# raynbowy23/RegT-GCN

Hardware: AMD Instinct MI355X
Metric: training steps/sec (graph-snapshots/sec) (higher is better)
Workload: dtype fp32; 1 GPU; cfg3: ONE synthetic regional graph, 100000 nodes / 1000000 edges / 8 regions, F=32, T=12, O=1, hidden=256; RegionalTemporalGCN forward+MSE+backward per snapshot, RMSprop step once per K steps (run.py semantics); gemm_arithmetic=fp32 MFMA (v_mfma_f32_32x32x2_f32), global_nodes=100000, global_edges=1000000, global_regions=8, parallelism=single GPU

## Files before the change

regt-gcn_amd/csrc/api.hip:

```cpp
#include <limits.h>
#include <stdarg.h>

#include <functional>
#include <initializer_list>
#include <map>
#include <mutex>
#include <string>
#include <unordered_map>
#include <vector>

#include "../../include/regtgcn.h"
#include <algorithm>
#include "kernels.h"

namespace regt {

static thread_local char g_err[512] = "";
void set_error(const char* fmt, ...) {
    va_list ap;
    va_start(ap, fmt);
    vsnprintf(g_err, sizeof(g_err), fmt, ap);
    va_end(ap);
}

// ... 976 lines not shown
    TRY(rq.flush());
    PROF("compose_bwd", st);
    {
        SgBatch b{};
        for (int k = 0; k < 3; ++k) {
            const float* dG = k < 2 ? L.dGzr + (long)k * C * F : L.dGh;
            const float* dc = k < 2 ? L.dczr + (long)k * C : L.dch;
            add_task(b, gr.gate_w[k], 2L * C, 1, 0, C, C, 1, nullptr, 0,
                     {term(dG, F, 1, 0, p.conv_lin_w[k], 1, F, 0, F), term(dc, 1, 0, 0, p.conv_bias[k], 0, 1, 0, 1)});
            add_task(b, gr.conv_lin_w[k], 1, F, 0, F, C, 1, nullptr, 0, {term(dG, 1, F, 0, p.gate_w[k], 2L * C, 1, 0, C)});
            add_task(b, gr.conv_bias[k], 1, 0, 0, C, 1, 1, nullptr, 0, {term(p.gate_w[k], 1, 2L * C, 0, dc, 1, 0, 0, C)});
        }
        for (int k = 0; k < 3; ++k)
            add_task(b, gr.gate_b[k], 1, 0, 0, C, 1, 1, k < 2 ? L.dczr + (long)k * C : L.dch, 1, {});
        if (tcol) {
            const float* dP0[2] = {L.dP01, L.dP01 + (long)C * 2 * F};
            const float* dP1[2] = {L.dP01 + F, L.dP01 + (long)C * 2 * F + F};
            const float* dc[2] = {L.dczr, L.dczr + C};
            for (int k = 0; k < 2; ++k)
                add_task(b, gr.gate_w[k] + C, 2L * C, 1, 0, C, C, 1, nullptr, 0,
                         {term(dP0[k], 2L * F, 1, 0, p.cheb_w0, 1, F, 0, F), term(dP1[k], 2L * F, 1, 0, p.cheb_w1, 1, F, 0, F),
                          term(dc[k], 1, 0, 0, p.cheb_bias, 0, 1, 0, 1)});
            add_task(b, gr.cheb_w0, 1, F, 0, F, C, 1, gr.cheb_w0, 1,
                     {term(dP0[0], 1, 2L * F, 0, p.gate_w[0] + C, 2L * C, 1, 0, C), term(dP0[1], 1, 2L * F, 0, p.gate_w[1] + C, 2L * C, 1, 0, C)}, F);
            add_task(b, gr.cheb_w1, 1, F, 0, F, C, 1, gr.cheb_w1, 1,
                     {term(dP1[0], 1, 2L * F, 0, p.gate_w[0] + C, 2L * C, 1, 0, C), term(dP1[1], 1, 2L * F, 0, p.gate_w[1] + C, 2L * C, 1, 0, C)}, F);
            add_task(b, gr.cheb_bias, 1, 0, 0, C, 1, 1, gr.cheb_bias, 1,
                     {term(p.gate_w[0] + C, 1, 2L * C, 0, dc[0], 1, 0, 0, C), term(p.gate_w[1] + C, 1, 2L * C, 0, dc[1], 1, 0, 0, C)});
        }
        if (d.regional) {
            const long RC = (long)R * C;
            int lo, hi;
            region_range(d, g, &lo, &hi);
            const SgTerm g0a = term(L.dA0, F, 1, 0, p.cheb_w0, 1, F, 0, F), g0b = term(L.dbprime, 1, 0, 0, p.cheb_bias, 0, 1, 0, 1);
            add_task(b, gr.region_w + (long)lo * C, RC, 1, C, C, C, hi - lo, nullptr, 0,
                     {g0a, g0b, term(L.dAall + (long)lo * C * F, F, 1, (long)C * F, p.cheb_w1, 1, F, 0, F)});
            if (lo > 0) add_task(b, gr.region_w, RC, 1, C, C, C, lo, nullptr, 0, {g0a, g0b});
            if (hi < R) add_task(b, gr.region_w + (long)hi * C, RC, 1, C, C, C, R - hi, nullptr, 0, {g0a, g0b});
            add_task(b, gr.cheb_w0, 1, F, 0, F, C, 1, nullptr, 0, {term(L.dA0, 1, F, 0, L.S, C, 1, 0, C)});
            add_task(b, gr.cheb_w1, 1, F, 0, F, C, 1, nullptr, 0,
                     {term(L.dAall + (long)lo * C * F, 1, F, (long)C * F, p.region_w + (long)lo * C, RC, 1, C, C, hi - lo, 1)});
            add_task(b, gr.cheb_bias, 1, 0, 0, C, 1, 1, nullptr, 0, {term(L.S, 1, C, 0, L.dbprime, 1, 0, 0, C)});
            add_task(b, gr.region_b, 1, 0, 0, C, 1, 1, L.dbprime, 1, {});
        }
        TRY(launch_small_gemm_multi(b, st));
    }
    return REGT_OK;
}

int check_ptrs(const regt_params* p, const regt_dims& d, bool cell_only = false) {
    REGT_CHECK_ARG(p != nullptr, "params is NULL");
    bool ok = p->attention && p->head1_w && p->head1_b && p->head2_w && p->head2_b;
    if (!cell_only) ok = ok && p->cheb_w0 && p->cheb_w1 && p->cheb_bias;
    for (int k = 0; k < 3; ++k) ok = ok && p->conv_lin_w[k] && p->conv_bias[k] && p->gate_w[k] && p->gate_b[k];
    if (d.regional && !cell_only) ok = ok && p->region_w && p->region_b;
    REGT_CHECK_ARG(ok, "params: a required tensor pointer is NULL");
    return REGT_OK;
}

}
}

using namespace regt;

extern "C" {

int32_t regt_abi_version(void) { return REGT_ABI_VERSION; }

int32_t regt_set_gemm_mode(int32_t mode) {
    const int prev = gemm_mode();
    set_gemm_mode(mode);
    return prev;
}
const char* regt_last_error(void) { return g_err; }

int32_t regt_set_option(const char* name, int32_t value) {
    REGT_CHECK_ARG(name != nullptr, "regt_set_option: name is NULL");
    if (!strcmp(name, "xbf")) { const int prev = xbf_wanted() ? 1 : 0; g_opt_xbf = value ? 1 : 0; return prev; }
    if (!strcmp(name, "fused_rows")) { const int prev = g_opt_fused_rows; g_opt_fused_rows = value == 2 ? 2 : (value ? 1 : 0); return prev; }
    if (!strcmp(name, "embed_kernel")) { const int prev = g_opt_embed_kernel; g_opt_embed_kernel = value ? 1 : 0; return prev; }
    if (!strcmp(name, "fused_bwd")) { const int prev = fused_bwd_wanted() ? 1 : 0; g_opt_fused_bwd = value ? 1 : 0; return prev; }
    if (!strcmp(name, "spmm_rows")) return spmm_rows_option(value);
    if (!strcmp(name, "dgrad1_gen")) return dgrad1_gen_option(value);
    if (!strcmp(name, "wgrad_ring")) return wgrad_ring_option(value);
    if (!strcmp(name, "wgrad_tile")) return wgrad_tile_option(value);
    if (!strcmp(name, "wgrad_ring256")) return wgrad_ring256_option(value == 4 ? 4 : 2);
    if (!strcmp(name, "wgrad_bnw64")) return wgrad_bnw64_option(value ? 1 : 0);
    if (!strcmp(name, "wgrad_wave")) return wgrad_wave_option(value ? 1 : 0);
    if (!strcmp(name, "wgrad_pairs")) { const int prev = wgrad_pairs_setting(); g_opt_wgrad_pairs = value < 0 || value > 2 ? 2 : value; return prev; }
    if (!strcmp(name, "tgcn_collapse")) { const int prev = tcollapse_wanted() ? 1 : 0; g_opt_tcollapse = value ? 1 : 0; return prev; }
    set_error("regt_set_option: unknown option '%s'", name);
    return -1;
}

size_t regt_graph_workspace_bytes(int64_t E, int32_t N) { return graph_workspace_bytes((long)E, N); }

int32_t regt_gcn_csr(const int64_t* ei, const float* w, int64_t E, int32_t N, int32_t* rowptr, int32_t* col, float* val,
                     int32_t* flags_dev, void* ws, size_t ws_bytes, regt_stream_t st) {
    REGT_CHECK_ARG((ei || E == 0) && rowptr && col && val && flags_dev && ws, "regt_gcn_csr: NULL pointer");
    return graph_gcn_csr(ei, w, (long)E, N, rowptr, col, val, flags_dev, ws, ws_bytes, (hipStream_t)st);
}

int32_t regt_gcn_dis(const int64_t* ei, const float* w, int64_t E, int32_t N, float* dis_out, int32_t* flags_dev, void* ws, size_t ws_bytes,
                     regt_stream_t st) {
    REGT_CHECK_ARG((ei || E == 0) && dis_out && flags_dev && ws, "regt_gcn_dis: NULL pointer");
    return graph_gcn_dis(ei, w, (long)E, N, dis_out, flags_dev, ws, ws_bytes, (hipStream_t)st);
}

int32_t regt_cheb_edge_weights(const int64_t* ei, const float* w, int64_t E, int32_t N, float* out, int32_t* flags_dev,
                               void* ws, size_t ws_bytes, regt_stream_t st) {
    REGT_CHECK_ARG((ei || E == 0) && (out || E == 0) && flags_dev && ws, "regt_cheb_edge_weights: NULL pointer");
    return graph_cheb_edge_weights(ei, w, (long)E, N, out, flags_dev, ws, ws_bytes, (hipStream_t)st);
}

int32_t regt_raw_csr(const int64_t* ei, const float* v, int64_t E, int32_t N, int32_t* rowptr, int32_t* col, float* val,
                     int32_t* flags_dev, void* ws, size_t ws_bytes, regt_stream_t st) {
    REGT_CHECK_ARG((ei || E == 0) && rowptr && col && val && flags_dev && ws, "regt_raw_csr: NULL pointer");
    return graph_raw_csr(ei, v, (long)E, N, rowptr, col, val, flags_dev, ws, ws_bytes, (hipStream_t)st);
}

int32_t regt_graph_fingerprint(const int64_t* ei, const float* w, int64_t E, uint64_t* out_dev, regt_stream_t st) {
    REGT_CHECK_ARG((ei || E == 0) && out_dev, "regt_graph_fingerprint: NULL pointer");
    return graph_fingerprint(ei, w, (long)E, reinterpret_cast<unsigned long long*>(out_dev), (hipStream_t)st);
}

int32_t regt_spmm_csr(const int32_t* rowptr, const int32_t* col, const float* val, const float* X, float* Y, int32_t nrows,
                      int32_t nrows_x, int32_t width, regt_stream_t st) {
    REGT_CHECK_ARG(rowptr && col && val && X && Y, "regt_spmm_csr: NULL pointer");
    return launch_spmm_csr(rowptr, col, val, X, Y, nrows, nrows_x, width, 1, (hipStream_t)st);
}

int32_t regt_spmm_dual(const int32_t* rowptr, const int32_t* col, const float* val_a, const float* val_l, const float* X,
                       float* YA, float* YL, int32_t N, int32_t width, regt_stream_t st) {
    REGT_CHECK_ARG(rowptr && col && val_a && val_l && X && YA && YL, "regt_spmm_dual: NULL pointer");
    return launch_spmm_dual(rowptr, col, val_a, val_l, X, YA, YL, N, width, (hipStream_t)st);
}

int32_t regt_pack_x(const float* x, float* xp, int32_t N, int32_t F, int32_t T, regt_stream_t st) {
    REGT_CHECK_ARG(x && xp && N > 0 && F > 0 && T > 0, "regt_pack_x: bad argument");
    return launch_pack_x(x, xp, N, F, T, (hipStream_t)st);
}

int32_t regt_linear(const float* A, int64_t lda, int64_t M, int32_t K, const float* W, int64_t ldw, int32_t N,
                    const float* bias, int32_t act, float slope, float* out, int64_t ldo, regt_stream_t st) {
    REGT_CHECK_ARG(A && W && out && M > 0 && K > 0 && N > 0, "regt_linear: bad argument");
    REGT_CHECK_ARG(act >= 0 && act <= 4, "regt_linear: act must be 0 (none), 1 (leaky_relu), 2 (relu), 3 (sigmoid) or 4 (tanh)");
    GemmSegs S{};
    S.nseg = 1;
    S.seg[0] = make_seg(A, lda, W, nullptr, ldw, INT_MAX, K, true);
    S.row_div = 1;
    EpiBiasAct e{out, ldo, bias, act, slope};
    return launch_gemm_bias_act(S, M, N, e, (hipStream_t)st);
}

static void wgrad_chunks(int64_t M, int* kchunk, int* nchunks) {
    long kc = ((M + 127) / 128 + 31) / 32 * 32;
    if (kc < 512) kc = 512;
    *kchunk = (int)kc;
    *nchunks = (int)((M + kc - 1) / kc);
}

size_t regt_wgrad_slab_floats(int64_t M, int32_t N, int32_t K, int32_t with_bias) {
    int kc, nc;
    wgrad_chunks(M, &kc, &nc);
    return (size_t)nc * ((size_t)N * K + (with_bias ? N : 0));
}
// ... 353 lines not shown
```

regt-gcn_amd/csrc/gemm.hip:

```cpp
#include "kernels.h"
#include "gemm_fast.h"
#include "gemm_split.h"
#include "gemm_small.h"

namespace regt {

#ifdef REGT_WG_TRACE
__device__ long g_wg_trace[4 * WG_TRACE_MAX];
__device__ long g_wg_marks[8 * WG_TRACE_MAX];
#define WG_TRACE_T(name) const long name = wall_clock64()
#define WG_TRACE_END(N, ta, tb)                                                                                              \
    if (threadIdx.x == 0 && WG_TILE_ID < WG_TRACE_MAX && (N) == REGT_WG_TRACE_N) {                                            \
        long* q_ = g_wg_trace + 4L * WG_TILE_ID;                                                                              \
        q_[0] = ta; q_[1] = tb; q_[2] = wall_clock64();                                                                       \
        q_[3] = ((long)__builtin_amdgcn_s_getreg((31 << 11) | 4)) | ((long)__builtin_amdgcn_s_getreg((31 << 11) | 20) << 32); \
    }
#else
#define WG_TRACE_T(name)
#define WG_TRACE_END(N, ta, tb)
#endif

__device__ __forceinline__ float fast_sigmoid(float x) { return __builtin_amdgcn_rcpf(1.0f + __expf(-x)); }
__device__ __forceinline__ float fast_tanh(float x) { return 1.0f - 2.0f * __builtin_amdgcn_rcpf(1.0f + __expf(2.0f * x)); }
__device__ __forceinline__ float4 ld4(const float* p) { return *reinterpret_cast<const float4*>(p); }
// ... 676 lines not shown
#pragma unroll
        for (int j = 0; j < 2; ++j)
#pragma unroll
            for (int r = 0; r < 16; ++r) acc[i][j][r] = 0.f;
    core.run(acc);
    if (vec) core.for_each_vec(acc, epi);
    else core.for_each(acc, [&](int r, int c, float v) { epi(m0 + r, c, v); });
}

template <class EpiF, class Core>
__global__ __launch_bounds__(256, 2) void gemm_flat_fast_kernel(GemmSegs S, long M, int N, EpiF epi, int relu_a) {
    extern __shared__ __attribute__((aligned(16))) float lds[];
    const int tiles_n = (N + GBN - 1) / GBN;
    const int bid = xcd_remap(blockIdx.x, gridDim.x);
    const long m0 = (long)(bid / tiles_n) * GBM;
    const int n0 = (bid % tiles_n) * GBN;
    RowMap rm{m0, 1, (int)((M - m0) < GBM ? (M - m0) : GBM)};
    Core core(S, rm, n0, N, lds);
    core.fill_rowtab(epi);
    core.plan();
    f32x16 acc[2][2];
#pragma unroll
    for (int i = 0; i < 2; ++i)
#pragma unroll
        for (int j = 0; j < 2; ++j)
#pragma unroll
            for (int r = 0; r < 16; ++r) acc[i][j][r] = 0.f;
    WG_TRACE_T(t_a);
    core.run(acc, relu_a != 0);
    WG_TRACE_T(t_b);
    core.for_each_vec(acc, epi);
    WG_TRACE_END(N, t_a, t_b);
}

template <class EpiF, bool REGION, int NP>
__global__ __launch_bounds__(256, 3) void gemm_flat_split_kernel(GemmSegs S, long M, int N, EpiF epi, int relu_a, int uniform) {
    extern __shared__ __attribute__((aligned(16))) float lds[];
    const int tiles_n = (N + GBN - 1) / GBN;
    const int bid = xcd_remap(blockIdx.x, gridDim.x);
    const long m0 = (long)(bid / tiles_n) * GBM;
    const int n0 = (bid % tiles_n) * GBN;
    RowMap rm{m0, 1, (int)((M - m0) < GBM ? (M - m0) : GBM)};
    WG_MARK(6);
    SplitCore<REGION, NP> core(S, rm, n0, N, lds, true);
    WG_MARK(7);
    core.fill_rowtab(epi);
    const bool uni = uniform != 0;
    if (!uni) core.plan();
    f32x16 acc[2][2];
#pragma unroll
    for (int i = 0; i < 2; ++i)
#pragma unroll
        for (int j = 0; j < 2; ++j)
#pragma unroll
            for (int r = 0; r < 16; ++r) acc[i][j][r] = 0.f;
    WG_TRACE_T(t_a);
    if (uni) core.run_uniform(acc, relu_a != 0);
    else core.run(acc, relu_a != 0);
    WG_TRACE_T(t_b);
    core.for_each_vec_halves(acc, epi);
    WG_TRACE_END(N, t_a, t_b);
}

template <int NP>
__global__ __launch_bounds__(256, 2) void gemm_dgrad1_gen_kernel(GemmSegs S, long M, int N, EpiDgrad1GenF epi) {
    extern __shared__ __attribute__((aligned(16))) float lds[];
    const int tiles_n = (N + GBN - 1) / GBN;
    const int bid = xcd_remap(blockIdx.x, gridDim.x);
    const long m0 = (long)(bid / tiles_n) * GBM;
    const int n0 = (bid % tiles_n) * GBN;
    RowMap rm{m0, 1, (int)((M - m0) < GBM ? (M - m0) : GBM)};
    SplitCore<false, NP> core(S, rm, n0, N, lds, true);
    core.fill_rowtab(epi);
    f32x16 acc[2][2];
#pragma unroll
    for (int i = 0; i < 2; ++i)
#pragma unroll
        for (int j = 0; j < 2; ++j)
#pragma unroll
            for (int r = 0; r < 16; ++r) acc[i][j][r] = 0.f;
    const typename SplitCore<false, NP>::AGen g{epi.e.ZR, epi.e.Ht, epi.e.dOH, epi.e.dhp, epi.e.C, (unsigned)epi.e.num_nodes * (unsigned)epi.e.C * 4u};
    core.run_u_gen(acc, g);
    core.for_each_vec_halves(acc, epi);
}

template <class EpiF8, bool REGION>
__global__ __launch_bounds__(256, 3) void gemm_flat_split8_kernel(GemmSegs S, long M, int N, EpiF8 epi, int uniform) {
    extern __shared__ __attribute__((aligned(16))) float lds[];
    const int tiles_n = (N + GBN - 1) / GBN;
    const int bid = xcd_remap(blockIdx.x, gridDim.x);
    const long m0 = (long)(bid / tiles_n) * GBM;
    const int n0 = (bid % tiles_n) * GBN;
    RowMap rm{m0, 1, (int)((M - m0) < GBM ? (M - m0) : GBM)};
    SplitCore<REGION, 1> core(S, rm, n0, N, lds, true);
    core.fill_rowtab(epi);
    const bool uni = uniform != 0;
    if (!uni) core.plan();
    f32x16 acc[2][2];
#pragma unroll
    for (int i = 0; i < 2; ++i)
#pragma unroll
        for (int j = 0; j < 2; ++j)
#pragma unroll
            for (int r = 0; r < 16; ++r) acc[i][j][r] = 0.f;
    WG_TRACE_T(t_a);
    if (uniform == 2) core.run_uniform_frag(acc, false);
    else if (uni) core.run_uniform(acc, false);
    else core.run(acc, false);
    WG_TRACE_T(t_b);
    core.for_each_vec8_halves(acc, epi);
    WG_TRACE_END(N, t_a, t_b);
}

template <class EpiF, bool BT, bool REGION>
__global__ __launch_bounds__(256, 4) void gemm_flat_small_kernel(GemmSegs S, long M, int N, EpiF epi, int relu_a) {
    extern __shared__ __attribute__((aligned(16))) float lds[];
    const int tiles_n = (N + SM_B - 1) / SM_B;
    const long m0 = (long)(blockIdx.x / tiles_n) * SM_B;
    const int n0 = (blockIdx.x % tiles_n) * SM_B;
    RowMap rm{m0, 1, (int)((M - m0) < SM_B ? (M - m0) : SM_B)};
    SmallCore<BT, REGION> core(S, rm, n0, N, lds);
    core.plan();
    f32x16 acc;
#pragma unroll
    for (int r = 0; r < 16; ++r) acc[r] = 0.f;
    core.run(acc, relu_a != 0);
    core.for_each_vec(acc, epi);
}

static int g_gemm_mode = -1;
static thread_local int t_gemm_mode = -1;
int gemm_mode_override(int mode) { const int prev = t_gemm_mode; t_gemm_mode = mode; return prev; }
int gemm_mode() {
    if (t_gemm_mode >= 0) return t_gemm_mode;
    if (g_gemm_mode < 0) {
        const char* e = getenv("REGT_GEMM_MODE");
        g_gemm_mode = 0;
        if (e && (!strcmp(e, "bf16x3") || !strcmp(e, "1"))) g_gemm_mode = 1;
        if (e && (!strcmp(e, "bf16") || !strcmp(e, "2"))) g_gemm_mode = 2;
    }
    return g_gemm_mode;
}
void set_gemm_mode(int m) { g_gemm_mode = (m == 1 || m == 2) ? m : 0; }
bool fp32_core_wide() {
    static int wide = -1;
    if (wide < 0) { const char* e = getenv("REGT_FP32_CORE"); wide = e && !strcmp(e, "wide") ? 1 : 0; }
    return wide == 1;
}

bool gemm_desc_table_forced() {
    static int force_table = -1;
    if (force_table < 0) { const char* e = getenv("REGT_GEMM_DESC"); force_table = e && !strcmp(e, "table") ? 1 : 0; }
    return force_table == 1;
}
static int uniform_ok(const GemmSegs& S, long M) {
    if (gemm_desc_table_forced()) return 0;
    int frag = 0;
    long slabs = 0;
    for (int s = 0; s < S.nseg; ++s) {
        const GemmSeg& g = S.seg[s];
        if (g.K % GBK != 0 || g.K <= 0) return 0;
        if ((g.flags & SEG_REGION) && (g.flags & SEG_A_BF16)) return 0;
        if (g.lda * 4 * (GBM + 1) >= (1L << 31) || g.ldb * 4 * (GBN + 1) >= (1L << 31)) return 0;
        if (g.flags & SEG_B_FRAG) ++frag;
        const long reps = (g.flags & SEG_REGION) ? std::min<long>(S.num_regions > 0 ? S.num_regions : 1, GBM / (S.row_div > 0 ? S.row_div : 1) + 2)
                                                 : ((g.flags & SEG_REPEAT) ? g.nrep : 1);
// ... 70 lines not shown
            else
                hipLaunchKernelGGL((gemm_flat_split_kernel<EpiF, REGION, 1>), dim3((unsigned)tiles), dim3(256), SplitGeom<1>::LDS_BYTES, st, S, M, N, f, relu, uniform_ok(S, M));
            REGT_CHECK_LAUNCH();
            return REGT_OK;
        }
    }
    return launch_fast_core<EpiF, FastCore<BT, REGION>>(S, M, N, f, relu, st);
}

template <class EpiF8, bool REGION>
static int launch_split8(const GemmSegs& S, long M, int N, EpiF8 f, hipStream_t st) {
    REGT_CHECK_ARG(gemm_mode() == 2 && N % 8 == 0, "gemm: bf16-stored activations need REGT_GEMM_MODE=bf16 and N %% 8 == 0");
    for (int q = 0; q < S.nseg; ++q)
        REGT_CHECK_ARG(!(S.seg[q].flags & SEG_B_FRAG) || uniform_ok(S, M) == 2, "gemm: fragment-order weights need every segment in that order and K %% 32 == 0");
    const long tiles = (long)cdiv(M, GBM) * cdiv(N, GBN);
    REGT_CHECK_ARG(tiles < (1L << 31), "gemm: too many tiles");
    hipLaunchKernelGGL((gemm_flat_split8_kernel<EpiF8, REGION>), dim3((unsigned)tiles), dim3(256), SplitGeom<1>::LDS_BYTES, st, S, M, N, f, uniform_ok(S, M));
    REGT_CHECK_LAUNCH();
    return REGT_OK;
}

template <class EpiF>
static int launch_flat(const GemmSegs& S, long M, int N, EpiF f, bool vec, hipStream_t st) {
    REGT_CHECK_ARG(M > 0 && N > 0, "gemm: empty problem M=%ld N=%d", M, N);
    for (int q = 0; q < S.nseg; ++q)
        REGT_CHECK_ARG(!(S.seg[q].flags & SEG_A_BF16), "gemm: a bf16-stored operand needs the bf16-operand vector path");
    long tiles = (long)cdiv(M, GBM) * cdiv(N, GBN);
    REGT_CHECK_ARG(tiles < (1L << 31), "gemm: too many tiles");
    static bool attr_done = false;
    if (int rc = set_lds_once(&gemm_flat_kernel<EpiF>, G_LDS_BYTES, &attr_done)) return rc;
    hipLaunchKernelGGL(gemm_flat_kernel<EpiF>, dim3((unsigned)tiles), dim3(256), G_LDS_BYTES, st, S, M, N, f, vec ? 1 : 0);
    REGT_CHECK_LAUNCH();
    return REGT_OK;
}


int launch_gemm_bias_act(const GemmSegs& S, long M, int N, const EpiBiasAct& e, hipStream_t st) {
    const bool vec = N % 4 == 0 && e.ldo % 4 == 0 && a16(e.out) && a16(e.bias);
    const int fc = fast_class(S, N, vec);
    if (e.out_bf16) {
        REGT_CHECK_ARG(fc >= 0 && (fc & 1) && !(fc & 4) && e.ldo % 8 == 0, "bias/act gemm: bf16 output needs the bf16-operand vector path");
        if (fc & 2) return launch_split8<EpiBiasAct8F, true>(S, M, N, EpiBiasAct8F{e}, st);
        return launch_split8<EpiBiasAct8F, false>(S, M, N, EpiBiasAct8F{e}, st);
    }
    if (fc >= 0 && (fc & 1)) {
        if (fc & 2) return launch_fast<EpiBiasActF, true, true>(S, M, N, EpiBiasActF{e}, (fc >> 2) & 1, st);
        return launch_fast<EpiBiasActF, true, false>(S, M, N, EpiBiasActF{e}, (fc >> 2) & 1, st);
    }
    return launch_flat(S, M, N, EpiBiasActF{e}, vec, st);
}
int launch_gemm_gates(const GemmSegs& S, long M, int N, const EpiGates& e, hipStream_t st) {
    REGT_CHECK_ARG(N == 2 * e.C, "gates gemm expects N == 2C");
    const bool vec = e.C % 4 == 0 && a16(e.ZR) && a16(e.h) && a16(e.q) && a16(e.bias);
    if (e.h_bf16 || e.zr_bf16) {
        REGT_CHECK_ARG(fast_class(S, N, vec) == 1 && e.C % 8 == 0, "gates gemm: bf16-stored activations need the bf16-operand vector path");
        return launch_split8<EpiGates8F, false>(S, M, N, EpiGates8F{e}, st);
    }
    if (fast_class(S, N, vec) == 1) return launch_fast<EpiGatesF, true, false>(S, M, N, EpiGatesF{e}, 0, st);
    REGT_CHECK_ARG(!e.q_bf16, "gates gemm: bf16 storage of q needs the vector path");
    return launch_flat(S, M, N, EpiGatesF{e}, vec, st);
}
int launch_gemm_dgrad1(const GemmSegs& S, long M, int N, const EpiDgrad1& e, hipStream_t st) {
    REGT_CHECK_ARG(N == e.C, "dgrad1 gemm expects N == C");
    const bool vec = e.C % 4 == 0 && a16(e.h) && a16(e.ZR) && a16(e.dOH) && a16(e.dzr) && a16(e.dh);
    if (e.h_bf16 || e.zr_bf16 || e.dh_bf16) {
        REGT_CHECK_ARG(fast_class(S, N, vec) == 1 && e.C % 8 == 0, "dgrad1 gemm: bf16-stored activations need the bf16-operand vector path");
        return launch_split8<EpiDgrad18F, false>(S, M, N, EpiDgrad18F{e}, st);
    }
    if (fast_class(S, N, vec) == 1) return launch_fast<EpiDgrad1F, true, false>(S, M, N, EpiDgrad1F{e}, 0, st);
    REGT_CHECK_ARG(!e.dzr_bf16, "dgrad1 gemm: bf16 storage of dzr needs the bf16-operand vector path");
    if (fast_class(S, N, vec) == 0) return launch_fast<EpiDgrad1F, false, false>(S, M, N, EpiDgrad1F{e}, 0, st);
    return launch_flat(S, M, N, EpiDgrad1F{e}, vec, st);
}
static int g_dgrad1_gen = -1;
static bool dgrad1_gen_wanted() {
    if (g_dgrad1_gen < 0) { const char* e = getenv("REGT_DGRAD1_GEN"); g_dgrad1_gen = e ? atoi(e) : 1; }
    return g_dgrad1_gen != 0;
}
int dgrad1_gen_option(int value) {
    const int prev = dgrad1_gen_wanted() ? 1 : 0;
    g_dgrad1_gen = value ? 1 : 0;
    return prev;
}
bool gemm_dgrad1_gen_ok(long M, int C, int num_nodes) {
    return dgrad1_gen_wanted() && (gemm_mode() == 0 || gemm_mode() == 1) && !fp32_core_wide() && !gemm_desc_table_forced() && C % GBN == 0 && C % GBK == 0 &&
           (long)cdiv(M, GBM) * (C / GBN) >= SMALL_TILE_LIMIT && M < (1L << 31) && (long)num_nodes * C * 4 < (1L << 31) &&
           (long)C * 8 * (GBM + 1) < (1L << 31);
}
int launch_gemm_dgrad1_gen(const GemmSegs& S, long M, int N, const EpiDgrad1& e, hipStream_t st) {
    REGT_CHECK_ARG(N == e.C && S.nseg == 1 && S.seg[0].K == e.C && (S.seg[0].flags & SEG_BT) && (S.seg[0].flags & SEG_VEC_B) &&
                   !(S.seg[0].flags & (SEG_A_BF16 | SEG_B_FRAG | SEG_REGION | SEG_REPEAT)), "dgrad1 (generated operand): one [N][K] weight segment with K = C");
    REGT_CHECK_ARG(gemm_dgrad1_gen_ok(M, e.C, e.num_nodes), "dgrad1 (generated operand): shape / arithmetic not covered");
    REGT_CHECK_ARG(e.Ht && e.dhp && e.rowdot && !e.dzr_bf16 && !e.h_bf16 && !e.zr_bf16 && !e.dh_bf16, "dgrad1 (generated operand): fp32 arrays, all outputs given");
    REGT_CHECK_ARG(a16(e.h) && a16(e.ZR) && a16(e.dOH) && a16(e.dzr) && a16(e.dh) && a16(e.Ht) && a16(e.dhp), "dgrad1 (generated operand): 16-byte aligned arrays");
    const long tiles = (long)cdiv(M, GBM) * (N / GBN);
    REGT_CHECK_ARG(tiles < (1L << 31), "gemm: too many tiles");
    if (gemm_mode() == 1)
        hipLaunchKernelGGL(gemm_dgrad1_gen_kernel<3>, dim3((unsigned)tiles), dim3(256), SplitGeom<3>::LDS_BYTES, st, S, M, N, EpiDgrad1GenF{e, e.C / GBN});
    else
        hipLaunchKernelGGL(gemm_dgrad1_gen_kernel<0>, dim3((unsigned)tiles), dim3(256), SplitGeom<0>::LDS_BYTES, st, S, M, N, EpiDgrad1GenF{e, e.C / GBN});
    REGT_CHECK_LAUNCH();
    return REGT_OK;
}
int launch_gemm_dgrad2(const GemmSegs& S, long M, int N, const EpiDgrad2& e, hipStream_t st) {
    REGT_CHECK_ARG(N == e.C, "dgrad2 gemm expects N == C");
    const bool vec = e.C % 4 == 0 && a16(e.dh) && a16(e.h);
    if (e.h_bf16 || e.dh_bf16) {
        REGT_CHECK_ARG(fast_class(S, N, vec) == 1 && e.C % 8 == 0, "dgrad2 gemm: bf16-stored activations need the bf16-operand vector path");
        return launch_split8<EpiDgrad28F, false>(S, M, N, EpiDgrad28F{e}, st);
    }
    if (fast_class(S, N, vec) == 1) return launch_fast<EpiDgrad2F, true, false>(S, M, N, EpiDgrad2F{e}, 0, st);
    if (fast_class(S, N, vec) == 0) return launch_fast<EpiDgrad2F, false, false>(S, M, N, EpiDgrad2F{e}, 0, st);
    return launch_flat(S, M, N, EpiDgrad2F{e}, vec, st);
}
int launch_gemm_mask_add(const GemmSegs& S, long M, int N, const EpiMaskAdd& e, hipStream_t st) {
    const bool vec = N % 4 == 0 && e.ldo % 4 == 0 && e.ldm % 4 == 0 && (!e.add || e.ldadd % 4 == 0) && a16(e.out) &&
                     a16(e.mask) && a16(e.add);
    if (fast_class(S, N, vec) == 0) return launch_fast<EpiMaskAddF, false, false>(S, M, N, EpiMaskAddF{e}, 0, st);
    return launch_flat(S, M, N, EpiMaskAddF{e}, vec, st);
}

__global__ __launch_bounds__(256, 1) void gemm_cand_kernel(CandArgs a) {
    extern __shared__ __attribute__((aligned(16))) float lds[];
    const int tiles_n = (a.C + GBN - 1) / GBN;
    const long C = a.C;
    f32x16 acc[2][2];
    const int bid = xcd_remap(blockIdx.x, gridDim.x);
    const int i0 = (bid / tiles_n) * GBM;
    const int n0 = (bid % tiles_n) * GBN;
    const int nvalid = (a.num_nodes - i0) < GBM ? (a.num_nodes - i0) : GBM;
    f32x16 oh[2][2];
#pragma unroll
    for (int i = 0; i < 2; ++i)
#pragma unroll
        for (int j = 0; j < 2; ++j)
#pragma unroll
            for (int r = 0; r < 16; ++r) oh[i][j][r] = 0.f;
    for (int t = 0; t < a.T; ++t) {
        RowMap rm{(long)i0 * a.T + t, a.T, nvalid};
        GemmCore core(a.S, rm, n0, a.C, lds);
#pragma unroll
        for (int i = 0; i < 2; ++i)
#pragma unroll
            for (int j = 0; j < 2; ++j)
#pragma unroll
                for (int r = 0; r < 16; ++r) acc[i][j][r] = 0.f;
        core.run(acc);
        const float pt = a.probs[t];
        core.for_each2(acc, oh, [&](int r, int c, float v, float o) {
            long m = rm.grow(r);
            float ht = fast_tanh(v + a.bias[c]);
            a.Ht[m * C + c] = ht;
            float Z = a.ZR[m * 2 * C + c];
            float hv = a.h[m * C + c];
            return o + pt * (Z * hv + (1.0f - Z) * ht);
        });
    }
    RowMap rm{(long)i0, 1, nvalid};
    GemmCore core(a.S, rm, n0, a.C, lds);
    core.for_each(oh, [&](int r, int c, float v) { a.OH[(long)(i0 + r) * C + c] = v; });
}

template <class Core>
__global__ __launch_bounds__(256, 2) void gemm_cand_flat_kernel(CandArgs a) {
    extern __shared__ __attribute__((aligned(16))) float lds[];
    constexpr int BM = Core::BM, BN = Core::BN, KROW = Core::EKROW, TPR = Core::ETPR;
    const long C = a.C, M = (long)a.num_nodes * a.T;
    const int tiles_n = (a.C + BN - 1) / BN;
    const int bid = xcd_remap(blockIdx.x, gridDim.x);
    const long m0 = (long)(bid / tiles_n) * BM;
    const int n0 = (bid % tiles_n) * BN;
    const RowMap rm{m0, 1, (int)((M - m0) < BM ? (M - m0) : BM)};
    Core core(a.S, rm, n0, a.C, lds);
    core.plan();
    typename Core::Acc acc;
    Core::zero(acc);
    core.run(acc, false);
    const int c = core.ecol();
    const int node0 = (int)(m0 / a.T);
    constexpr int RR = Core::EROWS >= 8 ? 8 : Core::EROWS;
// ... 601 lines not shown
```

regt-gcn_amd/csrc/kernels.h:

```cpp
#pragma once
#include "gemm_core.h"

namespace regt {
#ifdef REGT_WG_TRACE
#ifndef REGT_WG_TRACE_N
#define REGT_WG_TRACE_N 512
#endif
constexpr int WG_TRACE_MAX = 40000;
extern __device__ long g_wg_marks[8 * WG_TRACE_MAX];
#define WG_TILE_ID ((int)(rm.base / 128) * ((N + 127) / 128) + n0 / 128)
#define WG_MARK(i) do { if (threadIdx.x == 0 && WG_TILE_ID < WG_TRACE_MAX && N == REGT_WG_TRACE_N) g_wg_marks[8L * WG_TILE_ID + (i)] = wall_clock64(); } while (0)
#else
#define WG_MARK(i) do { } while (0)
#endif

typedef unsigned int u32x4_t __attribute__((ext_vector_type(4)));
typedef unsigned int u32x2_t __attribute__((ext_vector_type(2)));
__device__ __forceinline__ __amdgpu_buffer_rsrc_t buf_srd(const void* p) {
    const unsigned long long a = reinterpret_cast<unsigned long long>(p);
    const unsigned lo = __builtin_amdgcn_readfirstlane((unsigned)a);
    const unsigned hi = __builtin_amdgcn_readfirstlane((unsigned)(a >> 32));
    return __builtin_amdgcn_make_buffer_rsrc(reinterpret_cast<void*>(((unsigned long long)hi << 32) | lo), 0, 0x7FFFFFF0, 0x00020000);
}
__device__ __forceinline__ float4 buf_ld4(__amdgpu_buffer_rsrc_t r, int voff, int soff) {
    const u32x4_t v = __builtin_amdgcn_raw_buffer_load_b128(r, voff, soff, 0);
    return make_float4(__uint_as_float(v.x), __uint_as_float(v.y), __uint_as_float(v.z), __uint_as_float(v.w));
}
__device__ __forceinline__ void buf_st4(__amdgpu_buffer_rsrc_t r, int voff, int soff, float4 v) {
    const u32x4_t w = {__float_as_uint(v.x), __float_as_uint(v.y), __float_as_uint(v.z), __float_as_uint(v.w)};
    __builtin_amdgcn_raw_buffer_store_b128(w, r, voff, soff, 0);
}
__device__ __forceinline__ void buf_st4_bf16(__amdgpu_buffer_rsrc_t r, int voff, int soff, float4 v) {
    typedef __bf16 bf16x2_t __attribute__((ext_vector_type(2)));
    typedef float f32x2_t __attribute__((ext_vector_type(2)));
    const f32x2_t lo = {v.x, v.y}, hi = {v.z, v.w};
    const u32x2_t w = {__builtin_bit_cast(unsigned, __builtin_convertvector(lo, bf16x2_t)),
                       __builtin_bit_cast(unsigned, __builtin_convertvector(hi, bf16x2_t))};
    __builtin_amdgcn_raw_buffer_store_b64(w, r, voff, soff, 0);
}
__device__ __forceinline__ float gru_blend(float Z, float h, float ht) { return fmaf(Z, h, __fmul_rn(1.0f - Z, ht)); }
__device__ __forceinline__ float cb_dhp(float g, float z, float ht) { return __fmul_rn(__fmul_rn(g, 1.0f - z), fmaf(-ht, ht, 1.0f)); }
__device__ __forceinline__ float cb_dzp(float g, float h, float ht, float z) { return __fmul_rn(__fmul_rn(g, h - ht), __fmul_rn(z, 1.0f - z)); }
__device__ __forceinline__ float cb_drp(float dq, float h, float r) { return __fmul_rn(__fmul_rn(dq, h), __fmul_rn(r, 1.0f - r)); }
__device__ __forceinline__ float cb_dh(float dq, float r, float p, float d, float z) { return fmaf(dq, r, __fmul_rn(__fmul_rn(p, d), z)); }
__device__ __forceinline__ float cb_ds(float dh, float acc, float factor) { return __fmul_rn(dh + acc, factor); }

struct EpiRowEnt { int off; float p; };
struct EpiGeom { long m0; int n0, rr, c, step; const EpiRowEnt* rowtab; };
constexpr int EPI_ROWTAB_BYTES = 128 * (int)sizeof(EpiRowEnt);


enum : int { ACT_NONE = 0, ACT_LRELU = 1, ACT_RELU = 2, ACT_SIGMOID = 3, ACT_TANH = 4 };

struct EpiBiasAct {
    float* out; long ldo; const float* bias; int act; float slope;
    int out_bf16 = 0;
};
struct EpiGates {
    float* ZR;
    const float* h; float* q; const float* bias; int C;
    int q_bf16 = 0;
    int h_bf16 = 0, zr_bf16 = 0;
};
struct EpiDgrad1 {
    const float* h; const float* ZR; const float* dOH; const float* probs;
    float* dzr; float* dh; int C; int T;
    int dzr_bf16 = 0;
    int h_bf16 = 0, zr_bf16 = 0, dh_bf16 = 0;
    const float* Ht = nullptr; float* dhp = nullptr; float* rowdot = nullptr; int num_nodes = 0;
};
struct EpiDgrad2 {
    float* dh; const float* h; int C; int act; float slope;
    int h_bf16 = 0, dh_bf16 = 0;
};
struct EpiMaskAdd {
    float* out; long ldo; const float* mask; long ldm; const float* add; long ldadd;
};

int launch_gemm_bias_act(const GemmSegs& S, long M, int N, const EpiBiasAct& e, hipStream_t st);
int launch_gemm_gates(const GemmSegs& S, long M, int N, const EpiGates& e, hipStream_t st);
int launch_gemm_dgrad1(const GemmSegs& S, long M, int N, const EpiDgrad1& e, hipStream_t st);
bool gemm_dgrad1_gen_ok(long M, int C, int num_nodes);
int wgrad_bnw64_option(int value);
int wgrad_ring256_option(int value);
int wgrad_tile_option(int value);
int wgrad_wave_option(int value);
bool wgrad_ring_chunking(int Nout, int Nin, long M, int* kchunk, int* nchunks);
bool wgrad_skinny_chunking(int Nout, long M, int* kchunk, int* nchunks);
bool wgrad_wide_chunking(int Nout, int Nin, long M, int* kchunk, int* nchunks);
long wgrad_chunk_bound(int Nout, int Nin, long M);
bool wgrad_ring_active();
int wgrad_ring_option(int value);
int dgrad1_gen_option(int value);
int launch_gemm_dgrad1_gen(const GemmSegs& S, long M, int N, const EpiDgrad1& e, hipStream_t st);
int launch_gemm_dgrad2(const GemmSegs& S, long M, int N, const EpiDgrad2& e, hipStream_t st);
int launch_gemm_mask_add(const GemmSegs& S, long M, int N, const EpiMaskAdd& e, hipStream_t st);

struct CandArgs {
    GemmSegs S;
    int num_nodes, T, C;
    const float* bias;
    const float* ZR;
    const float* h;
    const float* probs;
    float* Ht;
    float* OH;
    int act_bf16 = 0;
    int node_sum_rows = 64;
};
int launch_gemm_candidate(const CandArgs& a, hipStream_t st);

struct WgradArgs {
    const float* P; long ldp; int Nout;
    const float* Q; long ldq; int Nin;
    int q_relu;
    long M;
    int kchunk;
    const int* chunk_tab;
    int nchunks;
    float* slab;
    int colsum;
    const float* Q2 = nullptr; long ldq2 = 0; int nin_split = 0;
    int p_bf16 = 0, q_bf16 = 0;
    int all_csum = 0;
};
int launch_wgrad(const WgradArgs& a, hipStream_t st);
long wgrad_slab_stride(const WgradArgs& a);

struct WgradReduceArgs {
    const float* slab; int nchunks; long slab_stride;
    long elem_offset;
    long slab_ld;
    int Nout, Nin;
    const int* chunk_group;
    int ngroups;
    int group_base;
    float* out; long ldo; long group_stride;
    float* colsum_out;
    long colsum_offset;
    int ncolsum;
    int accumulate;
};
int launch_wgrad_reduce(const WgradReduceArgs& a, hipStream_t st);
constexpr int WR_MAX_TASKS = 12;
struct WgradReduceBatch {
    int n;
    int block_start[WR_MAX_TASKS + 1];
    WgradReduceArgs t[WR_MAX_TASKS];
};
int launch_wgrad_reduce_multi(WgradReduceBatch& b, hipStream_t st);

struct SmallGemm {
    const float* A; long sai, sak, sab;
    const float* B; long sbk, sbj, sbb;
    float* C; long sci, scj, scb;
    int m, n, k, batch;
    int sum_batch;
    int accumulate;
};
int launch_small_gemm(const SmallGemm& g, hipStream_t st);

struct SgTerm {
    const float* A; const float* B;
    int sai, sak, sab, sbk, sbj, sbb;
    int k;
    short batch, sum_batch;
};
struct SgTask {
    float* C; const float* init;
    int sci, scj, scb, init_si, init_sj;
    int m, n;
    short nbatch, nterm;
    short split, pad_;
    SgTerm term[3];
};
constexpr int SG_MAX_TASKS = 19;
// ... 127 lines not shown
```

Before: 63.17 snapshots/s.

## Add row-slab dgrad1 generated-operand GEMM kernel covering full C=256 width

Adds a specialised backward dgrad1 kernel for C=256. Each workgroup owns 32 rows across all 256 output columns, so the generated A operand (dOH scaled by p, combined with Z and Ht) is built once per row instead of once per N-tile. It double-buffers LDS slabs, uses fp32 MFMA, and fuses the dzr, dh, dhp and rowdot epilogues in a single pass. The aim is to cut redundant operand generation and repeated reads of ZR, Ht and dOH, at the cost of small M tiles that reload the whole B matrix for every 32 rows, plus high register and LDS pressure.

```diff
diff --git a/regt-gcn_amd/csrc/api.hip b/regt-gcn_amd/csrc/api.hip
--- a/regt-gcn_amd/csrc/api.hip
+++ b/regt-gcn_amd/csrc/api.hip
@@ -1082,6 +1082,7 @@
     if (!strcmp(name, "fused_bwd")) { const int prev = fused_bwd_wanted() ? 1 : 0; g_opt_fused_bwd = value ? 1 : 0; return prev; }
     if (!strcmp(name, "spmm_rows")) return spmm_rows_option(value);
     if (!strcmp(name, "dgrad1_gen")) return dgrad1_gen_option(value);
+    if (!strcmp(name, "dgrad1_rows")) return dgrad1_rows_option(value);
     if (!strcmp(name, "wgrad_ring")) return wgrad_ring_option(value);
     if (!strcmp(name, "wgrad_tile")) return wgrad_tile_option(value);
     if (!strcmp(name, "wgrad_ring256")) return wgrad_ring256_option(value == 4 ? 4 : 2);
diff --git a/regt-gcn_amd/csrc/gemm.hip b/regt-gcn_amd/csrc/gemm.hip
--- a/regt-gcn_amd/csrc/gemm.hip
+++ b/regt-gcn_amd/csrc/gemm.hip
@@ -782,6 +782,143 @@
     const typename SplitCore<false, NP>::AGen g{epi.e.ZR, epi.e.Ht, epi.e.dOH, epi.e.dhp, epi.e.C, (unsigned)epi.e.num_nodes * (unsigned)epi.e.C * 4u};
     core.run_u_gen(acc, g);
     core.for_each_vec_halves(acc, epi);
+}
+
+namespace rows1 {
+constexpr int TM = 32;
+constexpr int C = 256;
+constexpr int NS = C / GBK;
+constexpr int ROW_B = GBK * 4;
+constexpr int A_B = TM * ROW_B, B_B = C * ROW_B, BUF_B = A_B + B_B;
+constexpr int IMG_LD = C + 4;
+constexpr int LDS_BYTES = 2 * BUF_B;
+static_assert(TM * IMG_LD * 4 <= BUF_B && TM * (C / 4) * 4 <= BUF_B, "epilogue images fit one slab buffer each");
+__device__ __forceinline__ constexpr int off(int r, int q) { return r * ROW_B + ((q ^ ((r >> 1) & 7)) << 4); }
+__device__ __forceinline__ float dot4(float4 d, float4 z, float4 h, float4 t) {
+    return (d.x * (z.x * h.x + (1.0f - z.x) * t.x) + d.y * (z.y * h.y + (1.0f - z.y) * t.y)) +
+           (d.z * (z.z * h.z + (1.0f - z.z) * t.z) + d.w * (z.w * h.w + (1.0f - z.w) * t.w));
+}
+}
+
+__global__ __launch_bounds__(256, 2) void gemm_dgrad1_gen_kernel_rows(GemmSegs S, long M, EpiDgrad1GenF epi) {
+    using namespace rows1;
+    extern __shared__ __attribute__((aligned(16))) float lds[];
+    char* lb = reinterpret_cast<char*>(lds);
+    const EpiDgrad1& e = epi.e;
+    const int tid = threadIdx.x, lane = tid & 63, w = tid >> 6, lr = lane & 31, lh = lane >> 5;
+    const long m0 = (long)xcd_remap(blockIdx.x, gridDim.x) * TM;
+    const int nvalid = (M - m0) < TM ? (int)(M - m0) : TM;
+    const int r = tid >> 3, q = tid & 7;
+    const long m = m0 + (r < nvalid ? r : 0);
+    const long node = m / e.T;
+    const float p = e.probs[(int)(m - node * e.T)];
+    const float* ZR = e.ZR + m0 * (2L * C);
+    const __amdgpu_buffer_rsrc_t sz = __builtin_amdgcn_make_buffer_rsrc(const_cast<float*>(ZR), 0, nvalid * C * 8, 0x00020000);
+    const __amdgpu_buffer_rsrc_t st = __builtin_amdgcn_make_buffer_rsrc(const_cast<float*>(e.Ht + m0 * C), 0, nvalid * C * 4, 0x00020000);
+    const __amdgpu_buffer_rsrc_t sd = __builtin_amdgcn_make_buffer_rsrc(const_cast<float*>(e.dOH), 0, (int)((unsigned)e.num_nodes * (unsigned)C * 4u), 0x00020000);
+    const __amdgpu_buffer_rsrc_t so = __builtin_amdgcn_make_buffer_rsrc(e.dhp + m0 * C, 0, nvalid * C * 4, 0x00020000);
+    const __amdgpu_buffer_rsrc_t sb = __builtin_amdgcn_make_buffer_rsrc(const_cast<float*>(S.seg[0].B0), 0, (int)(C * S.seg[0].ldb * 4), 0x00020000);
+    const int vz = r * C * 8 + q * 16, vt = r * C * 4 + q * 16, vd = (int)(node * C * 4) + q * 16;
+    const int vb = (tid >> 3) * (int)S.seg[0].ldb * 4 + q * 16, vbj = 32 * (int)S.seg[0].ldb * 4;
+
+    float4 z[NS], t[NS], d, b[8];
+    auto load_zt = [&](int s) {
+        z[s] = buf_ld4(sz, vz, s * ROW_B);
+        t[s] = buf_ld4(st, vt, s * ROW_B);
+    };
+    auto load = [&](int s) {
+        d = buf_ld4(sd, vd, s * ROW_B);
+#pragma unroll
+        for (int j = 0; j < 8; ++j) b[j] = buf_ld4(sb, vb + j * vbj, s * ROW_B);
+    };
+    auto stage = [&](int s) {
+        char* buf = lb + (s & 1) * BUF_B;
+        float4 a;
+        a.x = cb_dhp(__fmul_rn(p, d.x), z[s].x, t[s].x); a.y = cb_dhp(__fmul_rn(p, d.y), z[s].y, t[s].y);
+        a.z = cb_dhp(__fmul_rn(p, d.z), z[s].z, t[s].z); a.w = cb_dhp(__fmul_rn(p, d.w), z[s].w, t[s].w);
+        *reinterpret_cast<float4*>(buf + off(r, q)) = a;
+        buf_st4(so, vt + s * ROW_B, 0, a);
+#pragma unroll
+        for (int j = 0; j < 8; ++j) *reinterpret_cast<float4*>(buf + A_B + off((tid >> 3) + 32 * j, q)) = b[j];
+    };
+    f32x16 acc[2];
+#pragma unroll
+    for (int nt = 0; nt < 2; ++nt)
+#pragma unroll
+        for (int i = 0; i < 16; ++i) acc[nt][i] = 0.f;
+
+#pragma unroll
+    for (int s = 0; s < NS; ++s) load_zt(s);
+    load(0);
+    stage(0);
+    load(1);
+    __syncthreads();
+#pragma unroll
+    for (int s = 0; s < NS; ++s) {
+        const char* buf = lb + (s & 1) * BUF_B;
+#pragma unroll
+        for (int h = 0; h < 2; ++h) {
+            float4 fa[2], fb[2][2];
+#pragma unroll
+            for (int kk = 0; kk < 2; ++kk) {
+                fa[kk] = *reinterpret_cast<const float4*>(buf + off(lr, 4 * h + 2 * kk + lh));
+#pragma unroll
+                for (int nt = 0; nt < 2; ++nt)
+                    fb[nt][kk] = *reinterpret_cast<const float4*>(buf + A_B + off(64 * w + 32 * nt + lr, 4 * h + 2 * kk + lh));
+            }
+#pragma unroll
+            for (int kk = 0; kk < 2; ++kk)
+#pragma unroll
+                for (int j = 0; j < 4; ++j)
+#pragma unroll
+                    for (int nt = 0; nt < 2; ++nt)
+                        acc[nt] = __builtin_amdgcn_mfma_f32_32x32x2f32(reinterpret_cast<const float*>(&fa[kk])[j],
+                                                                      reinterpret_cast<const float*>(&fb[nt][kk])[j], acc[nt], 0, 0, 0);
+        }
+        if (s + 1 < NS) stage(s + 1);
+        if (s + 2 < NS) load(s + 2);
+        __syncthreads();
+    }
+
+    const __amdgpu_buffer_rsrc_t sh = __builtin_amdgcn_make_buffer_rsrc(const_cast<float*>(e.h + m0 * C), 0, nvalid * C * 4, 0x00020000);
+    float4 hv[NS], rv[NS];
+#pragma unroll
+    for (int s = 0; s < NS; ++s) {
+        hv[s] = buf_ld4(sh, vt, s * ROW_B);
+        rv[s] = buf_ld4(sz, vz, s * ROW_B + C * 4);
+    }
+    float* img = lds;
+    float* dots = reinterpret_cast<float*>(lb + BUF_B);
+#pragma unroll
+    for (int nt = 0; nt < 2; ++nt)
+#pragma unroll
+        for (int i = 0; i < 16; ++i) img[((i & 3) + 8 * (i >> 2) + 4 * lh) * IMG_LD + 64 * w + 32 * nt + lr] = acc[nt][i];
+    __syncthreads();
+    const __amdgpu_buffer_rsrc_t sdzr = __builtin_amdgcn_make_buffer_rsrc(e.dzr + m0 * (2L * C), 0, nvalid * C * 8, 0x00020000);
+    const __amdgpu_buffer_rsrc_t sdh = __builtin_amdgcn_make_buffer_rsrc(e.dh + m0 * C, 0, nvalid * C * 4, 0x00020000);
+#pragma unroll
+    for (int s = 0; s < NS; ++s) {
+        const float4 v = *reinterpret_cast<const float4*>(img + r * IMG_LD + 32 * s + 4 * q);
+        const float4 dd = buf_ld4(sd, vd, s * ROW_B), hh = hv[s], R = rv[s], Z = z[s], T = t[s];
+#define F_(k) cb_drp(v.k, hh.k, R.k)
+        buf_st4(sdzr, vz + s * ROW_B + C * 4, 0, REGT_V4(F_));
+#undef F_
+#define F_(k) cb_dh(v.k, R.k, p, dd.k, Z.k)
+        buf_st4(sdh, vt + s * ROW_B, 0, REGT_V4(F_));
+#undef F_
+#define F_(k) cb_dzp(__fmul_rn(p, dd.k), hh.k, T.k, Z.k)
+        buf_st4(sdzr, vz + s * ROW_B, 0, REGT_V4(F_));
+#undef F_
+        dots[r * (C / 4) + 8 * s + q] = dot4(dd, Z, hh, T);
+    }
+    __syncthreads();
+    const __amdgpu_buffer_rsrc_t srd = __builtin_amdgcn_make_buffer_rsrc(e.rowdot + m0 * (C / GBN), 0, nvalid * (C / GBN) * 4, 0x00020000);
+#pragma unroll
+    for (int i = 0; i < TM * (C / GBN) / 8; ++i) {
+        const int pr = 8 * i + (tid >> 5);
+        const float sum = EpiDgrad1GenF::half_wave_sum(dots[pr * 32 + (tid & 31)]);
+        if ((tid & 31) == EpiDgrad1GenF::SUM_LANE) __builtin_amdgcn_raw_buffer_store_b32(__float_as_uint(sum), srd, pr * 4, 0, 0);
+    }
 }
 
 template <class EpiF8, bool REGION>
@@ -1018,6 +1155,12 @@
     g_dgrad1_gen = value ? 1 : 0;
     return prev;
 }
+static int g_dgrad1_rows = 1;
+int dgrad1_rows_option(int value) {
+    const int prev = g_dgrad1_rows;
+    g_dgrad1_rows = value ? 1 : 0;
+    return prev;
+}
 bool gemm_dgrad1_gen_ok(long M, int C, int num_nodes) {
     return dgrad1_gen_wanted() && (gemm_mode() == 0 || gemm_mode() == 1) && !fp32_core_wide() && !gemm_desc_table_forced() && C % GBN == 0 && C % GBK == 0 &&
            (long)cdiv(M, GBM) * (C / GBN) >= SMALL_TILE_LIMIT && M < (1L << 31) && (long)num_nodes * C * 4 < (1L << 31) &&
@@ -1031,7 +1174,13 @@
     REGT_CHECK_ARG(a16(e.h) && a16(e.ZR) && a16(e.dOH) && a16(e.dzr) && a16(e.dh) && a16(e.Ht) && a16(e.dhp), "dgrad1 (generated operand): 16-byte aligned arrays");
     const long tiles = (long)cdiv(M, GBM) * (N / GBN);
     REGT_CHECK_ARG(tiles < (1L << 31), "gemm: too many tiles");
-    if (gemm_mode() == 1)
+    if (gemm_mode() == 0 && g_dgrad1_rows && e.C == rows1::C && S.seg[0].ldb == rows1::C && e.T > 0) {
+        static bool attr_done = false;
+        if (int rc = set_lds_once(&gemm_dgrad1_gen_kernel_rows, rows1::LDS_BYTES, &attr_done)) return rc;
+        const long rtiles = cdiv(M, rows1::TM);
+        REGT_CHECK_ARG(rtiles < (1L << 31), "gemm: too many tiles");
+        hipLaunchKernelGGL(gemm_dgrad1_gen_kernel_rows, dim3((unsigned)rtiles), dim3(256), rows1::LDS_BYTES, st, S, M, EpiDgrad1GenF{e, e.C / GBN});
+    } else if (gemm_mode() == 1)
         hipLaunchKernelGGL(gemm_dgrad1_gen_kernel<3>, dim3((unsigned)tiles), dim3(256), SplitGeom<3>::LDS_BYTES, st, S, M, N, EpiDgrad1GenF{e, e.C / GBN});
     else
         hipLaunchKernelGGL(gemm_dgrad1_gen_kernel<0>, dim3((unsigned)tiles), dim3(256), SplitGeom<0>::LDS_BYTES, st, S, M, N, EpiDgrad1GenF{e, e.C / GBN});
diff --git a/regt-gcn_amd/csrc/kernels.h b/regt-gcn_amd/csrc/kernels.h
--- a/regt-gcn_amd/csrc/kernels.h
+++ b/regt-gcn_amd/csrc/kernels.h
@@ -92,6 +92,7 @@
 bool wgrad_ring_active();
 int wgrad_ring_option(int value);
 int dgrad1_gen_option(int value);
+int dgrad1_rows_option(int value);
 int launch_gemm_dgrad1_gen(const GemmSegs& S, long M, int N, const EpiDgrad1& e, hipStream_t st);
 int launch_gemm_dgrad2(const GemmSegs& S, long M, int N, const EpiDgrad2& e, hipStream_t st);
 int launch_gemm_mask_add(const GemmSegs& S, long M, int N, const EpiMaskAdd& e, hipStream_t st);
```

After: 63.93 snapshots/s, median of 6. 1.2% higher.
